# TWeber132/thesis-clip-nerf

Hardware: AMD Instinct MI355X
Metric: rendered rays/sec (64 samples/ray) at 1/2/4/8 MI355X; RGB L1 vs ref (higher is better)
Workload: dtype f32

## Files before the change

### __graft_entry__.py

```python
import os
import subprocess
import sys

ROOT = os.path.dirname(os.path.abspath(__file__))
if ROOT not in sys.path:
    sys.path.insert(0, ROOT)


def build() -> None:
    csrc = os.path.join(ROOT, 'thesis_clip_nerf_amd', 'csrc')
    subprocess.run(['make', '-C', csrc], check=True)
    subprocess.run(['make', '-C', os.path.join(ROOT, 'tests', 'cpu_math')], check=True)
    import thesis_clip_nerf_amd
    from thesis_clip_nerf_amd import _lib
    assert _lib.lib().mvnerf_abi_version() == 1


def smoke() -> None:
    import numpy as np
    import torch

    from oracle import mvnerf_oracle as O
    from thesis_clip_nerf_amd import ops
    from thesis_clip_nerf_amd.synthetic import make_scene

    dev = torch.device('cuda:0')
    sc = make_scene(seed=11, height=16, width=16, n_views=1, n_rays=64, bias_scale=0.05)
    d = {k: torch.from_numpy(np.ascontiguousarray(sc[k])).to(dev) for k in
         ['rays_o', 'rays_d', 'images', 'features', 'intrinsics', 'extrinsics_inv', 'u_coarse', 'u_fine', 'coarse', 'fine']}
    ref = O.render_call(O.unflatten_net(sc['coarse']), O.unflatten_net(sc['fine']), sc['rays_o'], sc['rays_d'],
                        sc['images'], sc['intrinsics'], sc['extrinsics_inv'], sc['features'], sc['near'], sc['far'], 64,
                        sc['u_coarse'], sc['u_fine'])
    pc, pf = ops.pack_net(d['coarse']), ops.pack_net(d['fine'])
    split = (ops.pack_net_split(d['coarse']), ops.pack_net_split(d['fine']))
    for gemm, tables in (('split_f16', 'auto'), ('split_f16', None), ('split_bf16', 'auto'), ('split_bf16', None), ('mfma_f32', 'auto'), ('mfma_f32', None)):
# ... 26 lines not shown
```

### thesis_clip_nerf_amd/csrc/field_eval_split16_impl.h

```cpp
#include <hip/hip_runtime.h>

#include "mvnerf_field_common.h"
#include "mvnerf_kernels.h"
#include "mvnerf_launch.h"
#include "mvnerf_math.h"
#include "mvnerf_mfma.h"

#ifndef MVS16_F16
#error "include through field_eval_split16.hip / field_eval_split16h.hip"
#endif
#ifndef MVS16_GUARD
#define MVS16_GUARD 0
#endif
#if MVS16_GUARD && !MVS16_F16
#error "the range guard belongs to the fp16 form: the bf16 cut has the full fp32 range"
#endif
#if MVS16_GUARD
#define MVS16_LAUNCH_FN launch_field_eval_split16h_guard
#define MVS16_KERNEL field_eval_split16h_guard_kernel
#elif MVS16_F16
#define MVS16_BYTES packed_net_split16h_bytes
#define MVS16_PACK launch_pack_net_split16h
#define MVS16_SUPPORTS field_eval_split16h_supports
#define MVS16_LAUNCH_FN launch_field_eval_split16h
#define MVS16_KERNEL field_eval_split16h_kernel
#define MVS16_PACK_KERNEL pack_net_split16h_kernel
#else
#define MVS16_BYTES packed_net_split16_bytes
#define MVS16_PACK launch_pack_net_split16
#define MVS16_SUPPORTS field_eval_split16_supports
#define MVS16_LAUNCH_FN launch_field_eval_split16
#define MVS16_KERNEL field_eval_split16_kernel
#define MVS16_PACK_KERNEL pack_net_split16_kernel
#endif

namespace mvnerf {

namespace {

using f16x2 = __attribute__((ext_vector_type(2))) _Float16;

constexpr int kS16SlotChunks = 24;
constexpr int kS16L0Pe = 2, kS16L0Feat = 8, kS16Hidden = 48;
constexpr int kS16Steps = kS16L0Pe + kS16L0Feat + kS16Hidden;
constexpr int kS16Chunks = kS16Steps * kS16SlotChunks;
constexpr int kChunkElems16 = 512;

__host__ __device__ constexpr int s16_pe_row(int g, int e) {
    return g < 3 ? 20 * g + e : (e < 12 ? 20 * (e >> 2) + 2 * (8 + ((e >> 1) & 1)) + (e & 1) : (e < 15 ? 120 + (e - 12) : -1));
}

#if !MVS16_GUARD
__global__ void MVS16_PACK_KERNEL(const float* __restrict__ src, unsigned short* __restrict__ dst) {
    const int idx = blockIdx.x * blockDim.x + threadIdx.x;
    if (idx >= kS16Chunks * kChunkElems16) return;
    const int chunk = idx / kChunkElems16, lane = (idx % kChunkElems16) / 8, jj = idx % 8;
    const int i = lane & 15, g = lane >> 4;
    const int ks = chunk / kS16SlotChunks, rb = (chunk % kS16SlotChunks) / 3, piece = chunk % 3;
    float val = 0.0f;
    if (ks < kS16L0Pe) {
        const int row = s16_pe_row(g, 8 * ks + jj);
        if (row >= 0) val = src[kKerasW0 + row * kHidden + 16 * rb + i];
    } else if (ks < kS16L0Pe + kS16L0Feat) {
        const int row = 123 + 32 * (ks - kS16L0Pe) + 8 * g + jj;
        val = src[kKerasW0 + row * kHidden + 16 * rb + i];
    } else {
        const int q = ks - kS16L0Pe - kS16L0Feat, layer = q / 4, t = q % 4;
// ... 78 lines not shown
}

__device__ __forceinline__ void pin_pieces(B16& b, int q) {
#if MVS16_F16
    unsigned u1 = b.p1[q], u3 = b.p3[q];
    asm volatile("" : "+v"(u1), "+v"(u3));
    b.p1[q] = u1;
    b.p3[q] = u3;
#else
    unsigned u1 = b.p1[q], u2 = b.p2[q], u3 = b.p3[q];
    asm volatile("" : "+v"(u1), "+v"(u2), "+v"(u3));
    b.p1[q] = u1;
    b.p2[q] = u2;
    b.p3[q] = u3;
#endif
}

template <bool kRelu>
__device__ __forceinline__ void cut8(const float (&v)[8], B16& b, RangeMax& gm, int cb) {
#pragma unroll
    for (int q = 0; q < 4; ++q) cut_pair<kRelu>(v[2 * q], v[2 * q + 1], q, b, gm, cb);
}

constexpr int kR16Slots = 3, kR16SlotF4 = kS16SlotChunks * 64;
constexpr int kS16PerView = kS16Hidden / 2;
constexpr int kS16MaxPositions = 512;

struct Ring16 {
    const f32x4* w;
    unsigned char* lds;
    int cur, nxt, fill;
    const int* table;
    int pf4, P4;
    int start_pf;
    int lane_off, wave_off;
    u32x4 a0[3];
};

__device__ __forceinline__ int ring16_start_chunk(int p, int V, int l0_units) {
    const int per_view = l0_units + kS16PerView;
    if (p < per_view * V) {
        const int q = p % per_view;
        return (q < kS16L0Pe ? q : (q < l0_units ? q : kS16L0Pe + kS16L0Feat + (q - l0_units))) * kS16SlotChunks;
    }
    return (kS16L0Pe + kS16L0Feat + kS16PerView + (p - per_view * V)) * kS16SlotChunks;
}

constexpr int kR16DmaRequests = 3;
__device__ __forceinline__ void ring16_dma(const Ring16& r, int start, int slot) {
    const unsigned char* src = reinterpret_cast<const unsigned char*>(r.w) + (unsigned)start;
    const int dst = (int)(unsigned long)(__attribute__((address_space(3))) unsigned char*)r.lds + slot + r.wave_off;
    static_assert(kR16DmaRequests * 8192 == kS16SlotChunks * 1024, "a position is kR16DmaRequests requests of 8 KiB (8 waves x 1 KiB)");
#pragma unroll
    for (int i = 0; i < kR16DmaRequests; ++i)
        asm volatile("s_mov_b32 m0, %2\n\ts_nop 0\n\tglobal_load_lds_dwordx4 %0, %1" : : "v"(r.lane_off), "s"(src + 8192 * i), "s"(dst + 8192 * i) : "memory", "m0");
}

__device__ __forceinline__ void ring16_fetch(Ring16& r) {
    ring16_dma(r, __builtin_amdgcn_readfirstlane(r.start_pf), r.fill);
    r.start_pf = *reinterpret_cast<const int*>(reinterpret_cast<const unsigned char*>(r.table) + r.pf4);
    r.pf4 = r.pf4 + 4 == r.P4 ? 0 : r.pf4 + 4;
}

__device__ __forceinline__ const f32x4* ring16_cur(const Ring16& r) { return reinterpret_cast<const f32x4*>(r.lds + r.cur); }
__device__ __forceinline__ const f32x4* ring16_nxt(const Ring16& r) { return reinterpret_cast<const f32x4*>(r.lds + r.nxt); }

__device__ __forceinline__ void ring16_next(Ring16& r) {
    __builtin_amdgcn_s_waitcnt(0x0070);
    asm volatile("s_barrier" ::: "memory");
    const int done = r.cur;
    r.cur = r.nxt;
    r.nxt = r.fill;
    r.fill = done;
}

__device__ __forceinline__ int perm_f4(int rb, int g) {
    return ((g & 1) * 64 + (rb >> 1) * 16 + 4 * (2 * (rb & 1) + (g >> 1))) >> 2;
}

template <bool kAdd>
__device__ __forceinline__ void apply_bias_row(f32x4 (&row)[2], const f32x4& bv) {
#pragma unroll
    for (int cb = 0; cb < 2; ++cb)
#pragma unroll
        for (int c = 0; c < 4; ++c) {
            if (kAdd) {
                float r = row[cb][c];
                asm("v_add_f32_e32 %0, %1, %2" : "=v"(r) : "v"(r), "v"(bv[c]));
                row[cb][c] = r;
            } else {
                row[cb][c] = bv[c];
            }
        }
}

template <bool kRelu, int kMode, bool kTailAdd, bool kInit = false>
__device__ __forceinline__ void kstep16(Ring16& ring, int lane, int g, const B16 (&b)[2], const float (&nv)[2][8], B16 (&bn)[2], f32x4 (&acc)[8][2],
                                        f32x4 (&in)[8][2], const float* __restrict__ tail_bias, RangeMax& gm, const float* __restrict__ init_bias = nullptr,
                                        f32x4 init0 = f32x4{0.0f, 0.0f, 0.0f, 0.0f}) {
    const f32x4* cur = ring16_cur(ring) + lane;
    const f32x4* nxt = ring16_nxt(ring) + lane;
    u32x4 a[3] = {ring.a0[0], ring.a0[1], ring.a0[2]};
    f32x4 bv = {0.0f, 0.0f, 0.0f, 0.0f};
    int glane = (g & 1) * 16 + (g >> 1);
    if (kMode == 4 || kInit) asm volatile("" : "+v"(glane));
    const f32x4* tail_rows = reinterpret_cast<const f32x4*>(tail_bias) + glane;
    const f32x4* init_rows = reinterpret_cast<const f32x4*>(init_bias) + glane;
    f32x4 ci = init0;
#pragma unroll
    for (int rb = 0; rb < 8; ++rb) {
        u32x4 an[3];
#pragma unroll
        for (int q = 0; q < 3; ++q) an[q] = __builtin_bit_cast(u32x4, rb < 7 ? cur[((rb + 1) * 3 + q) * 64] : nxt[q * 64]);
        if (kMode == 1) cut_pair<kRelu>(nv[rb >> 2][2 * (rb & 3)], nv[rb >> 2][2 * (rb & 3) + 1], rb & 3, bn[rb >> 2], gm, rb >> 2);
        f32x4 cin = ci;
        if (kInit && rb < 7) cin = init_rows[((rb + 1) >> 1) * 4 + 2 * ((rb + 1) & 1)];
        if (kMode == 4 && tail_bias) {
            const f32x4 bv_new = tail_rows[(rb >> 1) * 4 + 2 * (rb & 1)];
            if (rb > 0) apply_bias_row<kTailAdd>(in[rb - 1], bv);
            bv = bv_new;
        }
#if MVS16_F16
#pragma unroll
        for (int cb = 0; cb < 2; ++cb) acc[rb][cb] = mfma1632(a[1], b[cb].p3, kInit ? ci : acc[rb][cb]);
#pragma unroll
        for (int cb = 0; cb < 2; ++cb) acc[rb][cb] = mfma1632(a[2], b[cb].p1, acc[rb][cb]);
#pragma unroll
        for (int cb = 0; cb < 2; ++cb) acc[rb][cb] = mfma1632(a[0], b[cb].p1, acc[rb][cb]);
#else
#pragma unroll
        for (int cb = 0; cb < 2; ++cb) acc[rb][cb] = mfma1632(a[2], b[cb].p1, kInit ? ci : acc[rb][cb]);
#pragma unroll
        for (int cb = 0; cb < 2; ++cb) acc[rb][cb] = mfma1632(a[1], b[cb].p2, acc[rb][cb]);
#pragma unroll
        for (int cb = 0; cb < 2; ++cb) acc[rb][cb] = mfma1632(a[0], b[cb].p3, acc[rb][cb]);
#pragma unroll
        for (int cb = 0; cb < 2; ++cb) acc[rb][cb] = mfma1632(a[1], b[cb].p1, acc[rb][cb]);
#pragma unroll
        for (int cb = 0; cb < 2; ++cb) acc[rb][cb] = mfma1632(a[0], b[cb].p2, acc[rb][cb]);
#pragma unroll
        for (int cb = 0; cb < 2; ++cb) acc[rb][cb] = mfma1632(a[0], b[cb].p1, acc[rb][cb]);
#endif
        __builtin_amdgcn_sched_group_barrier(0x008, 1, 0);
        __builtin_amdgcn_sched_group_barrier(0x100, (kMode == 4 || kInit) ? 4 : 3, 0);
#pragma unroll
        for (int m = 0; m < (MVS16_F16 ? 5 : 11); ++m) {
            if (kMode == 1) __builtin_amdgcn_sched_group_barrier(0x002, MVS16_F16 ? 2 : 1, 0);
            if (kMode == 4) __builtin_amdgcn_sched_group_barrier(0x002, MVS16_F16 ? 2 : 1, 0);
            __builtin_amdgcn_sched_group_barrier(0x008, 1, 0);
        }
        if (kMode == 1) __builtin_amdgcn_sched_group_barrier(0x002, MVS16_F16 ? 3 : 2, 0);
        __builtin_amdgcn_sched_barrier(0);
        if (rb == 0) {
            asm volatile("" : "+v"(acc[0][0]), "+v"(acc[0][1]));
            ring16_fetch(ring);
            __builtin_amdgcn_sched_barrier(0);
        }
#pragma unroll
        for (int q = 0; q < 3; ++q) a[q] = an[q];
        ci = cin;
    }
#pragma unroll
    for (int q = 0; q < 3; ++q) ring.a0[q] = a[q];
    if (kMode == 4 && tail_bias) apply_bias_row<kTailAdd>(in[7], bv);
    if (kMode == 1) {
#pragma unroll
        for (int cb = 0; cb < 2; ++cb)
#pragma unroll
            for (int q = 0; q < 4; ++q) {
                pin_pieces(bn[cb], q);
            }
    }
}

__device__ __forceinline__ void first_operand_s16(const f32x4 (&in)[8][2], B16 (&b)[2], RangeMax& gm) {
#pragma unroll
    for (int cb = 0; cb < 2; ++cb) {
        const float v8[8] = {in[0][cb][0], in[0][cb][1], in[0][cb][2], in[0][cb][3], in[1][cb][0], in[1][cb][1], in[1][cb][2], in[1][cb][3]};
        cut8<true>(v8, b[cb], gm, cb);
    }
}

template <bool kTailAdd, bool kInit>
__device__ __forceinline__ void dense128_s16_plain(Ring16& ring, int lane, int g, f32x4 (&in)[8][2], f32x4 (&acc)[8][2], const float* __restrict__ tail_bias,
                                                   RangeMax& gm, const float* __restrict__ init_bias = nullptr) {
    B16 b[2], bn[2];
    f32x4 init0 = {0.0f, 0.0f, 0.0f, 0.0f};
    if (kInit) init0 = reinterpret_cast<const f32x4*>(init_bias)[perm_f4(0, g)];
    first_operand_s16(in, b, gm);
#pragma unroll
    for (int t = 0; t < 4; ++t) {
        float nv[2][8];
#pragma unroll
        for (int cb = 0; cb < 2; ++cb)
#pragma unroll
            for (int q = 0; q < 8; ++q) nv[cb][q] = t < 3 ? in[2 * (t + 1) + (q >> 2)][cb][q & 3] : 0.0f;
        if (t == 0 && kInit) kstep16<true, 1, false, true>(ring, lane, g, b, nv, bn, acc, in, nullptr, gm, init_bias, init0);
        else if (t < 3) kstep16<true, 1, false>(ring, lane, g, b, nv, bn, acc, in, nullptr, gm);
        else kstep16<true, 4, kTailAdd>(ring, lane, g, b, nv, bn, acc, in, tail_bias, gm);
        b[0] = bn[0];
        b[1] = bn[1];
        ring16_next(ring);
    }
}

template <bool kAdd>
__device__ __forceinline__ void bias16(const float* __restrict__ bperm, int g, f32x4 (&acc)[8][2]) {
    int glane = (g & 1) * 16 + (g >> 1);
    asm volatile("" : "+v"(glane));
    const f32x4* p = reinterpret_cast<const f32x4*>(bperm) + glane;
#pragma unroll
    for (int rb = 0; rb < 8; ++rb) {
        const f32x4 v = p[(rb >> 1) * 4 + 2 * (rb & 1)];
#pragma unroll
        for (int cb = 0; cb < 2; ++cb)
#pragma unroll
            for (int c = 0; c < 4; ++c) {
                if (kAdd) {
                    float r = acc[rb][cb][c];
                    asm("v_add_f32_e32 %0, %1, %2" : "=v"(r) : "v"(r), "v"(v[c]));
                    acc[rb][cb][c] = r;
                } else {
                    acc[rb][cb][c] = v[c];
                }
            }
    }
}

constexpr int kS16StageRowBytes = 256;

__device__ __forceinline__ void store_tl16(float* __restrict__ base, long tile, int n, int g, const f32x4 (&x)[8][2]) {
    const __amdgpu_buffer_rsrc_t rsrc = __builtin_amdgcn_make_buffer_rsrc(base, 0, 0xFFFFFFFF, 0x00020000);
    const int voff = (4 * g * 32 + n) * 4;
    const int tile_off = (int)((unsigned)tile * 16384u);
#pragma unroll
    for (int rb = 0; rb < 8; ++rb)
#pragma unroll
        for (int i = 0; i < 4; ++i)
#pragma unroll
            for (int cb = 0; cb < 2; ++cb) {
                const float val = x[rb][cb][i];
                __builtin_amdgcn_raw_buffer_store_b32(__builtin_bit_cast(unsigned int, val), rsrc, voff + (i * 32 + 16 * cb) * 4,
                                                      tile_off + rb * 2048, kStashAux);
            }
}

struct SampleGeo {
    long g;
    int ray, sidx, b;
    float wx, wy, wz;
    bool valid;
};

template <bool kMultiView, bool kProj, bool kAux, bool kStash>
__global__ __launch_bounds__(512, 2) void MVS16_KERNEL(FieldParams p, const f32x4* __restrict__ wsplit
#if MVS16_GUARD
                                                       , unsigned* __restrict__ range_status
#endif
) {
    constexpr int kW = 8;
    extern __shared__ __attribute__((aligned(16))) unsigned char smem_s16[];
    constexpr int kRingBytes = kR16Slots * kR16SlotF4 * 16;
    const int tid = threadIdx.x, lane = tid & 63, n = lane & 15, g = lane >> 4;
    const int wave = __builtin_amdgcn_readfirstlane(tid >> 6);
    unsigned char* stage = smem_s16 + kRingBytes + wave * (32 * kS16StageRowBytes);
    float* net = reinterpret_cast<float*>(smem_s16 + kRingBytes + kW * 32 * kS16StageRowBytes) - kPackB0;
    for (int i = tid; i < kPackBr + 8 - kPackB0; i += 64 * kW) net[kPackB0 + i] = p.net[kPackB0 + i];
    int* table = reinterpret_cast<int*>(smem_s16 + kRingBytes + kW * 32 * kS16StageRowBytes + (kPackBr + 8 - kPackB0) * 4);
    float* wr_plain = reinterpret_cast<float*>(table + kS16MaxPositions);
    for (int i = tid; i < 512; i += 64 * kW) wr_plain[i] = p.net[kPackWrPlain + i];

    Ring16 ring;
    ring.w = wsplit;
    ring.lds = smem_s16;
    ring.cur = 0;
    ring.nxt = kR16SlotF4 * 16;
    ring.fill = 2 * kR16SlotF4 * 16;
    const int l0_units = kProj ? kS16L0Pe : kS16L0Pe + kS16L0Feat;
    const int n_pos = (l0_units + kS16PerView) * p.V + kS16PerView;
    for (int i = tid; i < n_pos; i += 64 * kW) table[i] = ring16_start_chunk(i, p.V, l0_units) * 1024;
    ring.table = table;
    ring.P4 = 4 * n_pos;
    ring.pf4 = 4 * 3;
    __syncthreads();
    ring.lane_off = 16 * tid;
    ring.wave_off = 1024 * wave;
    constexpr bool kSeedHere = !kMultiView && !kAux && !kStash;
    float* seed_w = reinterpret_cast<float*>(smem_s16 + kRingBytes);
    if (kSeedHere) {
        static_assert(kPackTotal - kPackW0Dir >= 8192 && kPackB0Plain + 128 - kPackW0Dir <= 8192 && kW * 32 * kS16StageRowBytes >= 32768,
                      "four 8 KiB requests: inside the packed net, covering W0_dir and b0, inside the gather stages");
        const unsigned char* src = reinterpret_cast<const unsigned char*>(p.net + kPackW0Dir);
        const int dst = (int)(unsigned long)(__attribute__((address_space(3))) unsigned char*)seed_w + ring.wave_off;
#pragma unroll
        for (int i = 0; i < 4; ++i)
            asm volatile("s_mov_b32 m0, %2\n\ts_nop 0\n\tglobal_load_lds_dwordx4 %0, %1" : : "v"(ring.lane_off), "s"(src + 8192 * i), "s"(dst + 8192 * i) : "memory", "m0");
    }
    ring16_dma(ring, __builtin_amdgcn_readfirstlane(table[0]), ring.cur);
    ring16_dma(ring, __builtin_amdgcn_readfirstlane(table[1]), ring.nxt);
    ring.start_pf = table[2];
    if (kSeedHere) asm volatile("s_waitcnt vmcnt(%0)" : : "n"(2 * kR16DmaRequests) : "memory");
    else asm volatile("s_waitcnt vmcnt(0)" ::: "memory");
    __syncthreads();
    if (kSeedHere) {
        const unsigned last_sample = (unsigned)p.total - 1u, S = (unsigned)p.S, R = (unsigned)p.R;
        const int groups = ((int)p.n_tiles + kW - 1) / kW;
        int turn = 0;
#pragma unroll 1
        for (int grp = blockIdx.x; grp < groups; grp += gridDim.x) {
            const unsigned first = (unsigned)grp * (32u * kW), end = first + (32u * kW - 1u);
            const int ray_hi = __builtin_amdgcn_readfirstlane((int)((end < last_sample ? end : last_sample) / S));
#pragma unroll 1
            for (int ray = __builtin_amdgcn_readfirstlane((int)(first / S)); ray <= ray_hi; ++ray, ++turn)
                if ((turn & (kW - 1)) == wave) {
                    const int b = __builtin_amdgcn_readfirstlane((int)((unsigned)ray / R));
                    dir_seed_row(p, b, ray - b * (int)R, lane, seed_w);
                }
        }
        asm volatile("s_waitcnt vmcnt(0)" ::: "memory");
        __syncthreads();
    }
#pragma unroll
    for (int q = 0; q < 3; ++q) ring.a0[q] = __builtin_bit_cast(u32x4, ring16_cur(ring)[q * 64 + lane]);

    RangeMax gm;
#if MVS16_GUARD
    gm.all = 0u;
#endif
    const int n_tiles = (int)p.n_tiles, n_groups = (n_tiles + kW - 1) / kW;
    for (int grp = blockIdx.x; grp < n_groups; grp += gridDim.x) {
        const int own = grp * kW + wave;
        const bool tile_ok = own < n_tiles;
        const long tile = tile_ok ? own : n_tiles - 1;
        int pS = p.S, pR = p.R, pH = p.H, pW = p.W, gl = g, nl = n;
        asm volatile("" : "+s"(pS), "+s"(pR), "+s"(pH), "+s"(pW));
        asm volatile("" : "+v"(gl), "+v"(nl));
        SampleGeo sg[2];
        const bool one_ray = (pS & 31) == 0;
        if (one_ray) {
            const unsigned first = (unsigned)tile * 32u;
            const int ray = __builtin_amdgcn_readfirstlane((int)(first / (unsigned)pS));
            const int b = __builtin_amdgcn_readfirstlane((int)((unsigned)ray / (unsigned)pR));
            const int s0 = (int)first - ray * pS;
            const cfloat* ro = (const cfloat*)(p.rays_o + 3 * ray);
            const cfloat* rd = (const cfloat*)(p.rays_d + 3 * ray);
            const float ox = ro[0], oy = ro[1], oz = ro[2], dx = rd[0], dy = rd[1], dz = rd[2];
#pragma unroll
            for (int cb = 0; cb < 2; ++cb) {
                const long gi = (long)first + 16 * cb + nl;
                sg[cb].valid = tile_ok;
                sg[cb].g = gi;
                sg[cb].ray = ray;
                sg[cb].sidx = s0 + 16 * cb + nl;
                sg[cb].b = b;
                const float zz = p.z[gi];
                sg[cb].wx = ox + zz * dx;
// ... 6 lines not shown
                long gi = tile * 32 + 16 * cb + nl;
                sg[cb].valid = tile_ok && gi < p.total;
                if (gi >= p.total) gi = p.total - 1;
                sg[cb].g = gi;
                const int ray = (int)((unsigned)gi / (unsigned)pS);
                sg[cb].ray = ray;
                sg[cb].sidx = (int)gi - ray * pS;
                sg[cb].b = (int)((unsigned)ray / (unsigned)pR);
                const float ox = p.rays_o[3 * ray + 0], oy = p.rays_o[3 * ray + 1], oz = p.rays_o[3 * ray + 2];
                const float dx = p.rays_d[3 * ray + 0], dy = p.rays_d[3 * ray + 1], dz = p.rays_d[3 * ray + 2];
                const float zz = p.z[gi];
                sg[cb].wx = ox + zz * dx;
                sg[cb].wy = oy + zz * dy;
                sg[cb].wz = oz + zz * dz;
            }
        }

        f32x4 x[8][2], hid[8][2];
        f32x4 xsum[kMultiView ? 8 : 1][2];
#if MVS16_GUARD
        gm.cb[0] = gm.cb[1] = 0u;
#endif

        const int n_views = (kMultiView || !(kAux || kStash)) ? p.V : 1;
        for (int v = 0; v < n_views; ++v) {
            asm volatile("" : "+s"(pS), "+s"(pR), "+s"(pH), "+s"(pW));
#pragma unroll
            for (int cb = 0; cb < 2; ++cb) asm volatile("" : "+v"(sg[cb].b), "+v"(sg[cb].ray), "+v"(sg[cb].sidx));
            int tl[2];
            float ax[2], ay[2];
            long vrow[2];
            float pe[2][16];
#pragma unroll
            for (int cb = 0; cb < 2; ++cb) {
                const int bv = sg[cb].b * p.V + v;
                float cam[4], pxl, pyl;
                const f32x4* seed;
                if (one_ray) {
                    const int bu = __builtin_amdgcn_readfirstlane(sg[0].b), bvu = bu * p.V + v;
                    const int rayu = __builtin_amdgcn_readfirstlane(sg[0].ray);
                    const cfloat* Ec = (const cfloat*)(p.einv + 16 * bvu);
                    const cfloat* Kc = (const cfloat*)(p.k4 + 16 * bvu);
                    float E[16], K[12];
#pragma unroll
                    for (int i = 0; i < 16; ++i) E[i] = Ec[i];
#pragma unroll
                    for (int i = 0; i < 12; ++i) K[i] = Kc[i];
// ... 64 lines not shown
                            const float a = img[c] * 2.0f - 1.0f, bq = img[3 + c] * 2.0f - 1.0f;
                            const float cq = img[3 * pW + c] * 2.0f - 1.0f, dq = img[3 * pW + 3 + c] * 2.0f - 1.0f;
                            vb[12 + c] = bilerp(a, bq, cq, dq, tp.ax, tp.ay);
                        }
                        vb[15] = 0.0f;
                    }
#pragma unroll
                    for (int e = 0; e < 16; ++e) pe[cb][e] = gl < 3 ? va[e] : vb[e];
                }
            }

            {
                B16 bq[2], bqn[2];
#pragma unroll
                for (int cb = 0; cb < 2; ++cb) {
                    const float v8[8] = {pe[cb][0], pe[cb][1], pe[cb][2], pe[cb][3], pe[cb][4], pe[cb][5], pe[cb][6], pe[cb][7]};
                    cut8<false>(v8, bq[cb], gm, cb);
                }
                float nv[2][8];
#pragma unroll
                for (int cb = 0; cb < 2; ++cb)
#pragma unroll
                    for (int q = 0; q < 8; ++q) nv[cb][q] = pe[cb][8 + q];
                kstep16<false, 1, false>(ring, lane, g, bq, nv, bqn, x, x, nullptr, gm);
                ring16_next(ring);
                kstep16<false, 0, false>(ring, lane, g, bqn, nv, bq, x, x, nullptr, gm);
                ring16_next(ring);
            }

            asm volatile("" : "+v"(gl), "+v"(nl));
#pragma unroll
            for (int P = 0; P < (kProj ? 2 : 4); ++P) {
                asm volatile("s_waitcnt lgkmcnt(0)" ::: "memory");
                const f32x4* tbase = kProj ? reinterpret_cast<const f32x4*>(p.texel_table) + (nl >> 3) * 16 + (nl & 7) + P * 8
                                           : reinterpret_cast<const f32x4*>(p.features) + P * 16 + nl;
                const long row_f4 = kProj ? 32 : 64;
#pragma unroll
                for (int half = 0; half < 2; ++half) {
                    f32x4 tv[4][4];
                    float axs[4], ays[4];
#pragma unroll
                    for (int u = 0; u < 4; ++u) {
                        const int src = 4 * u + gl;
                        const int tls = __shfl(tl[half], src);
                        axs[u] = __shfl(ax[half], src);
                        ays[u] = __shfl(ay[half], src);
                        const f32x4* f = tbase + (long)tls * row_f4;
                        tv[u][0] = f[0];
                        tv[u][1] = f[row_f4];
                        tv[u][2] = f[(long)pW * row_f4];
                        tv[u][3] = f[(long)pW * row_f4 + row_f4];
                    }
                    __builtin_amdgcn_sched_barrier(0);
#pragma unroll
                    for (int u = 0; u < 4; ++u) {
                        const int src = 16 * half + 4 * u + gl;
                        f32x4 o;
#pragma unroll
                        for (int c = 0; c < 4; ++c) {
                            const float top = fmaf(axs[u], tv[u][1][c] - tv[u][0][c], tv[u][0][c]);
                            const float bot = fmaf(axs[u], tv[u][3][c] - tv[u][2][c], tv[u][2][c]);
                            o[c] = fmaf(ays[u], bot - top, top);
                        }
                        *reinterpret_cast<f32x4*>(stage + src * kS16StageRowBytes + ((nl ^ (src & 15)) << 4)) = o;
                    }
                }
                asm volatile("s_waitcnt lgkmcnt(0)" ::: "memory");
                if (kProj) {
#pragma unroll
                    for (int cb = 0; cb < 2; ++cb)
#pragma unroll
                        for (int rbl = 0; rbl < 4; ++rbl) {
                            const int row = 16 * cb + nl, chunk = 8 * (gl & 1) + 4 * (rbl >> 1) + 2 * (rbl & 1) + (gl >> 1);
                            const f32x4 t4 = *reinterpret_cast<const f32x4*>(stage + row * kS16StageRowBytes + ((chunk ^ (row & 15)) << 4));
#pragma unroll
                            for (int c = 0; c < 4; ++c) x[4 * P + rbl][cb][c] += t4[c];
                        }
                } else {
#pragma unroll
                    for (int s = 0; s < 2; ++s) {
                        B16 bq[2], bqn[2];
                        float nv[2][8];
#pragma unroll
                        for (int cb = 0; cb < 2; ++cb) {
                            const int row = 16 * cb + nl;
                            const f32x4 lo = *reinterpret_cast<const f32x4*>(stage + row * kS16StageRowBytes + (((8 * s + 2 * gl) ^ (row & 15)) << 4));
                            const f32x4 hi = *reinterpret_cast<const f32x4*>(stage + row * kS16StageRowBytes + (((8 * s + 2 * gl + 1) ^ (row & 15)) << 4));
                            const float b8[8] = {lo[0], lo[1], lo[2], lo[3], hi[0], hi[1], hi[2], hi[3]};
                            cut8<false>(b8, bq[cb], gm, cb);
#pragma unroll
                            for (int q = 0; q < 8; ++q) nv[cb][q] = 0.0f;
                        }
                        kstep16<false, 0, false>(ring, lane, gl, bq, nv, bqn, x, x, nullptr, gm);
                        ring16_next(ring);
                    }
                }
            }

            const long vslot = (long)p.B * p.V * p.R * p.S * 128;
            const long vtile = kMultiView ? ((long)(sg[0].b * p.V + v) * (p.n_tiles / p.B) + (tile - (long)sg[0].b * (p.n_tiles / p.B))) : tile;
            if (kStash && tile_ok) store_tl16(p.stash, vtile, n, g, x);
            auto store_acc16 = [&](float* base, const long (&rows)[2]) {
#pragma unroll
                for (int cb = 0; cb < 2; ++cb)
                    if (sg[cb].valid) {
                        float* e = base + 128 * rows[cb] + 4 * g;
#pragma unroll
                        for (int rb = 0; rb < 8; ++rb) *reinterpret_cast<f32x4*>(e + 16 * rb) = x[rb][cb];
                    }
            };
            if (kAux && p.acts_view) store_acc16(p.acts_view, vrow);
#pragma unroll 1
            for (int bi = 0; bi < 3; ++bi) {
                const float* bias1 = net + kPackBHidden + 256 * bi;
                dense128_s16_plain<true, true>(ring, lane, g, x, hid, nullptr, gm, bias1);
                if (kStash && tile_ok) store_tl16(p.stash + (1 + 2 * bi) * p.stash_stride, vtile, n, g, hid);
                bias16<true>(bias1 + 128, g, x);
                dense128_s16_plain<false, false>(ring, lane, g, hid, x, nullptr, gm);
                if (kStash && tile_ok && bi < 2) store_tl16(p.stash + (2 + 2 * bi) * p.stash_stride, vtile, n, g, x);
                if (kAux && p.acts_view) store_acc16(p.acts_view + (bi + 1) * vslot, vrow);
            }
            if (kMultiView) {
#pragma unroll
                for (int rb = 0; rb < 8; ++rb)
#pragma unroll
                    for (int cb = 0; cb < 2; ++cb) xsum[rb][cb] = (v == 0) ? x[rb][cb] : xsum[rb][cb] + x[rb][cb];
            }
        }
        if (kMultiView) {
            const float nvw = (float)p.V;
#pragma unroll
            for (int rb = 0; rb < 8; ++rb)
#pragma unroll
                for (int cb = 0; cb < 2; ++cb) x[rb][cb] = xsum[rb][cb] / nvw;
        }

        long grow[2];
        bool gvalid[2];
        {
            int ne = n;
            asm volatile("" : "+v"(ne));
#pragma unroll
            for (int cb = 0; cb < 2; ++cb) {
                long gi = tile * 32 + 16 * cb + ne;
                gvalid[cb] = tile_ok && gi < p.total;
                grow[cb] = gi >= p.total ? p.total - 1 : gi;
            }
        }
        auto store_fused16 = [&](float* base) {
#pragma unroll
            for (int cb = 0; cb < 2; ++cb)
                if (gvalid[cb]) {
                    float* e = base + 128 * grow[cb] + 4 * g;
#pragma unroll
                    for (int rb = 0; rb < 8; ++rb) *reinterpret_cast<f32x4*>(e + 16 * rb) = x[rb][cb];
                }
        };
        if (kAux && p.acts_fused) store_fused16(p.acts_fused);
        if (kStash && tile_ok) store_tl16(p.stash_fused, tile, n, g, x);
#pragma unroll 1
        for (int bi = 3; bi < 6; ++bi) {
            const float* bias1 = net + kPackBHidden + 256 * bi;
            dense128_s16_plain<true, true>(ring, lane, g, x, hid, nullptr, gm, bias1);
            if (kStash && tile_ok) store_tl16(p.stash_fused + (1 + 2 * (bi - 3)) * p.stash_fused_stride, tile, n, g, hid);
            bias16<true>(bias1 + 128, g, x);
            dense128_s16_plain<false, false>(ring, lane, g, hid, x, nullptr, gm);
            if (kStash && tile_ok) store_tl16(p.stash_fused + (2 + 2 * (bi - 3)) * p.stash_fused_stride, tile, n, g, x);
            if (kAux && p.acts_fused) store_fused16(p.acts_fused + (long)(bi - 2) * p.total * 128);
        }
        if (kAux && p.embedding) store_fused16(p.embedding);

        {
            float o[2][4] = {{0.0f, 0.0f, 0.0f, 0.0f}, {0.0f, 0.0f, 0.0f, 0.0f}};
            const f32x4* wr = reinterpret_cast<const f32x4*>(wr_plain) + 4 * g;
#pragma unroll
            for (int rb = 0; rb < 8; ++rb)
#pragma unroll
                for (int c = 0; c < 4; ++c) {
                    const f32x4 w4 = wr[16 * rb + c];
#pragma unroll
                    for (int cb = 0; cb < 2; ++cb) {
                        const float a = fmaxf(x[rb][cb][c], 0.0f);
#pragma unroll
                        for (int k = 0; k < 4; ++k) o[cb][k] = fmaf(a, w4[k], o[cb][k]);
                    }
                }
#pragma unroll
            for (int cb = 0; cb < 2; ++cb)
#pragma unroll
// ... 18 lines not shown
        }
#if MVS16_GUARD
        {
            const unsigned m0 = gvalid[0] ? gm.cb[0] : 0u, m1 = gvalid[1] ? gm.cb[1] : 0u;
            gm.all = gm.all > m0 ? gm.all : m0;
            gm.all = gm.all > m1 ? gm.all : m1;
        }
#endif
    }
    asm volatile("s_waitcnt vmcnt(0)" ::: "memory");
#if MVS16_GUARD
    {
        unsigned m = gm.all;
#pragma unroll
        for (int off = 32; off >= 1; off >>= 1) {
            const unsigned o = (unsigned)__shfl_xor((int)m, off);
            m = m > o ? m : o;
        }
        if (lane == 0) *reinterpret_cast<unsigned*>(stage) = m;
        __syncthreads();
        if (tid == 0) {
            unsigned wg = 0u;
            for (int w = 0; w < kW; ++w) {
                const unsigned o = *reinterpret_cast<const unsigned*>(smem_s16 + kRingBytes + w * (32 * kS16StageRowBytes));
                wg = wg > o ? wg : o;
            }
            atomicMax(range_status, wg);
        }
    }
#endif
}

}

#if !MVS16_GUARD
size_t MVS16_BYTES() { return (size_t)kS16Chunks * 1024; }

hipError_t MVS16_PACK(const float* net_keras, void* packed_split16, hipStream_t st) {
    const int n = kS16Chunks * kChunkElems16;
    hipLaunchKernelGGL(MVS16_PACK_KERNEL, dim3((n + 255) / 256), dim3(256), 0, st, net_keras, static_cast<unsigned short*>(packed_split16));
    return hipGetLastError();
}

bool MVS16_SUPPORTS(const FieldParams& p) {
    if (p.stash && (p.tap_idx || p.pix || p.embedding || p.acts_view || p.acts_fused)) return false;
    const int n_pos = ((p.texel_table ? kS16L0Pe : kS16L0Pe + kS16L0Feat) + kS16PerView) * p.V + kS16PerView;
    return n_pos <= kS16MaxPositions;
}
#endif

#if MVS16_GUARD
hipError_t MVS16_LAUNCH_FN(const FieldParams& p, const void* packed_split16, float* range_status, hipStream_t stream) {
    static DeviceSetup setup;
    if (!range_status || !field_eval_split16h_supports(p)) return hipErrorInvalidValue;
    unsigned* status = reinterpret_cast<unsigned*>(range_status);
#else
hipError_t MVS16_LAUNCH_FN(const FieldParams& p, const void* packed_split16, hipStream_t stream) {
    static DeviceSetup setup;
    if (!MVS16_SUPPORTS(p)) return hipErrorInvalidValue;
#endif
    const int lds_bytes = kR16Slots * kR16SlotF4 * 16 + 8 * 32 * kS16StageRowBytes + (kPackBr + 8 - kPackB0) * 4 + kS16MaxPositions * 4 + 512 * 4;
    int cus = 0;
    hipError_t e = device_setup(setup, {{&MVS16_KERNEL<false, false, false, false>, lds_bytes}, {&MVS16_KERNEL<false, true, false, false>, lds_bytes},
                                        {&MVS16_KERNEL<true, false, false, false>, lds_bytes}, {&MVS16_KERNEL<true, true, false, false>, lds_bytes},
                                        {&MVS16_KERNEL<false, false, true, false>, lds_bytes}, {&MVS16_KERNEL<false, true, true, false>, lds_bytes},
                                        {&MVS16_KERNEL<true, false, true, false>, lds_bytes}, {&MVS16_KERNEL<true, true, true, false>, lds_bytes},
                                        {&MVS16_KERNEL<false, false, false, true>, lds_bytes}, {&MVS16_KERNEL<false, true, false, true>, lds_bytes},
                                        {&MVS16_KERNEL<true, false, false, true>, lds_bytes}, {&MVS16_KERNEL<true, true, false, true>, lds_bytes}}, &cus);
    if (e != hipSuccess) return e;
    const bool mv = p.V > 1;
    const bool aux = p.tap_idx || p.pix || p.embedding || p.acts_view || p.acts_fused;
    if ((mv || aux || p.stash) && (e = launch_dir_bias(p, stream)) != hipSuccess) return e;
    const long n_groups = (p.n_tiles + 7) / 8;
    const long resident = (long)cus;
    const unsigned wgs = (unsigned)(n_groups < resident ? n_groups : resident);
    const f32x4* w = static_cast<const f32x4*>(packed_split16);
    const dim3 grid(wgs), block(512);
#if MVS16_GUARD
#define MVS16_LAUNCH(MV, PROJ, AUX, STASH) hipLaunchKernelGGL((MVS16_KERNEL<MV, PROJ, AUX, STASH>), grid, block, lds_bytes, stream, p, w, status)
#else
#define MVS16_LAUNCH(MV, PROJ, AUX, STASH) hipLaunchKernelGGL((MVS16_KERNEL<MV, PROJ, AUX, STASH>), grid, block, lds_bytes, stream, p, w)
#endif
    if (p.stash && p.V > 1 && ((long)p.R * p.S) % 32 != 0) return hipErrorInvalidValue;
    if (p.stash) {
// ... 26 lines not shown
```

Measured before the change: 4.749 million.

## Pair ring positions to halve weight-ring barriers in split16 kernel

```diff
diff --git a/__graft_entry__.py b/__graft_entry__.py
--- a/__graft_entry__.py
+++ b/__graft_entry__.py
@@ -11,6 +11,7 @@
     csrc = os.path.join(ROOT, 'thesis_clip_nerf_amd', 'csrc')
     subprocess.run(['make', '-C', csrc], check=True)
     subprocess.run(['make', '-C', os.path.join(ROOT, 'tests', 'cpu_math')], check=True)
+    subprocess.run(['make', '-C', os.path.join(ROOT, 'tests', 'cpu_ring')], check=True)
     import thesis_clip_nerf_amd
     from thesis_clip_nerf_amd import _lib
     assert _lib.lib().mvnerf_abi_version() == 1
diff --git a/thesis_clip_nerf_amd/csrc/field_eval_split16_impl.h b/thesis_clip_nerf_amd/csrc/field_eval_split16_impl.h
--- a/thesis_clip_nerf_amd/csrc/field_eval_split16_impl.h
+++ b/thesis_clip_nerf_amd/csrc/field_eval_split16_impl.h
@@ -5,6 +5,7 @@
 #include "mvnerf_launch.h"
 #include "mvnerf_math.h"
 #include "mvnerf_mfma.h"
+#include "mvnerf_ring_pairs.h"
 
 #ifndef MVS16_F16
 #error "include through field_eval_split16.hip / field_eval_split16h.hip"
@@ -43,6 +44,8 @@
 constexpr int kS16SlotChunks = 24;
 constexpr int kS16L0Pe = 2, kS16L0Feat = 8, kS16Hidden = 48;
 constexpr int kS16Steps = kS16L0Pe + kS16L0Feat + kS16Hidden;
+static_assert(kS16L0Pe % 2 == 0 && kS16L0Feat % 2 == 0 && (kS16Hidden / 2) % 2 == 0,
+              "ring positions come in pairs: layer 0's PE and feature k-steps and the k-steps of a view's blocks are all even, so every tile is");
 constexpr int kS16Chunks = kS16Steps * kS16SlotChunks;
 constexpr int kChunkElems16 = 512;
 
@@ -167,16 +170,29 @@
     for (int q = 0; q < 4; ++q) cut_pair<kRelu>(v[2 * q], v[2 * q + 1], q, b, gm, cb);
 }
 
-constexpr int kR16Slots = 3, kR16SlotF4 = kS16SlotChunks * 64;
+constexpr int kR16Slots = kRingPairSlots, kR16SlotF4 = kS16SlotChunks * 64;
+constexpr int kR16SlotBytes = kR16SlotF4 * 16;
 constexpr int kS16PerView = kS16Hidden / 2;
 constexpr int kS16MaxPositions = 512;
+
+constexpr int kS16Waves = 8;
+constexpr int kS16StageRowBytes = 256;
+constexpr int kS16StageBytes = 16 * kS16StageRowBytes;
+constexpr int kS16LdsRing = 0, kS16RingBytes = kR16Slots * kR16SlotBytes;
+constexpr int kS16LdsStage = kS16LdsRing + kS16RingBytes;
+constexpr int kS16LdsNet = kS16LdsStage + kS16Waves * kS16StageBytes;
+constexpr int kS16LdsTable = kS16LdsNet + (kPackBr + 8 - kPackB0) * 4;
+constexpr int kS16LdsWr = kS16LdsTable + kS16MaxPositions * 4;
+constexpr int kS16LdsBytes = kS16LdsWr + 512 * 4;
+static_assert(kS16LdsBytes <= 160 * 1024, "ring, gather stages, biases, position table and read-out kernel share the compute unit's 160 KiB");
+static_assert(kS16LdsStage % 16 == 0 && kS16LdsNet % 16 == 0 && kS16LdsTable % 4 == 0 && kS16LdsWr % 16 == 0, "vector accesses are aligned");
 
 struct Ring16 {
     const f32x4* w;
     unsigned char* lds;
-    int cur, nxt, fill;
+    RingSlots s;
     const int* table;
-    int pf4, P4;
+    RingCursor c;
     int start_pf;
     int lane_off, wave_off;
     u32x4 a0[3];
@@ -193,31 +209,32 @@
 
 constexpr int kR16DmaRequests = 3;
 __device__ __forceinline__ void ring16_dma(const Ring16& r, int start, int slot) {
-    const unsigned char* src = reinterpret_cast<const unsigned char*>(r.w) + (unsigned)start;
-    const int dst = (int)(unsigned long)(__attribute__((address_space(3))) unsigned char*)r.lds + slot + r.wave_off;
+    const unsigned char* src = reinterpret_cast<const unsigned char*>(r.w) + (unsigned)(start + r.wave_off);
+    const int dst = __builtin_amdgcn_readfirstlane((int)(unsigned long)(__attribute__((address_space(3))) unsigned char*)r.lds + slot + r.wave_off);
     static_assert(kR16DmaRequests * 8192 == kS16SlotChunks * 1024, "a position is kR16DmaRequests requests of 8 KiB (8 waves x 1 KiB)");
 #pragma unroll
     for (int i = 0; i < kR16DmaRequests; ++i)
         asm volatile("s_mov_b32 m0, %2\n\ts_nop 0\n\tglobal_load_lds_dwordx4 %0, %1" : : "v"(r.lane_off), "s"(src + 8192 * i), "s"(dst + 8192 * i) : "memory", "m0");
 }
 
-__device__ __forceinline__ void ring16_fetch(Ring16& r) {
-    ring16_dma(r, __builtin_amdgcn_readfirstlane(r.start_pf), r.fill);
-    r.start_pf = *reinterpret_cast<const int*>(reinterpret_cast<const unsigned char*>(r.table) + r.pf4);
-    r.pf4 = r.pf4 + 4 == r.P4 ? 0 : r.pf4 + 4;
-}
-
-__device__ __forceinline__ const f32x4* ring16_cur(const Ring16& r) { return reinterpret_cast<const f32x4*>(r.lds + r.cur); }
-__device__ __forceinline__ const f32x4* ring16_nxt(const Ring16& r) { return reinterpret_cast<const f32x4*>(r.lds + r.nxt); }
-
-__device__ __forceinline__ void ring16_next(Ring16& r) {
+__device__ __forceinline__ void ring16_fetch(Ring16& r, bool second) {
+    ring16_dma(r, __builtin_amdgcn_readfirstlane(r.start_pf), ring_slots_fill(r.s, second, kR16SlotBytes));
+    r.start_pf = *reinterpret_cast<const int*>(reinterpret_cast<const unsigned char*>(r.table) + ring_cursor_take(r.c));
+}
+
+__device__ __forceinline__ const f32x4* ring16_cur(const Ring16& r, bool second) {
+    return reinterpret_cast<const f32x4*>(r.lds + (ring_slots_cur(r.s, second, kR16SlotBytes) + r.lane_off));
+}
+__device__ __forceinline__ const f32x4* ring16_nxt(const Ring16& r, bool second) {
+    return reinterpret_cast<const f32x4*>(r.lds + (ring_slots_nxt(r.s, second, kR16SlotBytes) + r.lane_off));
+}
+
+__device__ __forceinline__ void ring16_rendezvous() {
     __builtin_amdgcn_s_waitcnt(0x0070);
     asm volatile("s_barrier" ::: "memory");
-    const int done = r.cur;
-    r.cur = r.nxt;
-    r.nxt = r.fill;
-    r.fill = done;
-}
+}
+
+__device__ __forceinline__ void ring16_next(Ring16& r, bool second) { ring_slots_advance(r.s, second); }
 
 __device__ __forceinline__ int perm_f4(int rb, int g) {
     return ((g & 1) * 64 + (rb >> 1) * 16 + 4 * (2 * (rb & 1) + (g >> 1))) >> 2;
@@ -239,12 +256,12 @@
         }
 }
 
-template <bool kRelu, int kMode, bool kTailAdd, bool kInit = false>
-__device__ __forceinline__ void kstep16(Ring16& ring, int lane, int g, const B16 (&b)[2], const float (&nv)[2][8], B16 (&bn)[2], f32x4 (&acc)[8][2],
+template <bool kPairEnd, bool kRelu, int kMode, bool kTailAdd, bool kInit = false>
+__device__ __forceinline__ void kstep16(Ring16& ring, int g, const B16 (&b)[2], const float (&nv)[2][8], B16 (&bn)[2], f32x4 (&acc)[8][2],
                                         f32x4 (&in)[8][2], const float* __restrict__ tail_bias, RangeMax& gm, const float* __restrict__ init_bias = nullptr,
                                         f32x4 init0 = f32x4{0.0f, 0.0f, 0.0f, 0.0f}) {
-    const f32x4* cur = ring16_cur(ring) + lane;
-    const f32x4* nxt = ring16_nxt(ring) + lane;
+    const f32x4* cur = ring16_cur(ring, kPairEnd);
+    const f32x4* nxt = ring16_nxt(ring, kPairEnd);
     u32x4 a[3] = {ring.a0[0], ring.a0[1], ring.a0[2]};
     f32x4 bv = {0.0f, 0.0f, 0.0f, 0.0f};
     int glane = (g & 1) * 16 + (g >> 1);
@@ -254,6 +271,10 @@
     f32x4 ci = init0;
 #pragma unroll
     for (int rb = 0; rb < 8; ++rb) {
+        if (kPairEnd && rb == 7) {
+            ring16_rendezvous();
+            __builtin_amdgcn_sched_barrier(0);
+        }
         u32x4 an[3];
 #pragma unroll
         for (int q = 0; q < 3; ++q) an[q] = __builtin_bit_cast(u32x4, rb < 7 ? cur[((rb + 1) * 3 + q) * 64] : nxt[q * 64]);
@@ -298,7 +319,7 @@
         __builtin_amdgcn_sched_barrier(0);
         if (rb == 0) {
             asm volatile("" : "+v"(acc[0][0]), "+v"(acc[0][1]));
-            ring16_fetch(ring);
+            ring16_fetch(ring, kPairEnd);
             __builtin_amdgcn_sched_barrier(0);
         }
 #pragma unroll
@@ -327,7 +348,7 @@
 }
 
 template <bool kTailAdd, bool kInit>
-__device__ __forceinline__ void dense128_s16_plain(Ring16& ring, int lane, int g, f32x4 (&in)[8][2], f32x4 (&acc)[8][2], const float* __restrict__ tail_bias,
+__device__ __forceinline__ void dense128_s16_plain(Ring16& ring, int g, f32x4 (&in)[8][2], f32x4 (&acc)[8][2], const float* __restrict__ tail_bias,
                                                    RangeMax& gm, const float* __restrict__ init_bias = nullptr) {
     B16 b[2], bn[2];
     f32x4 init0 = {0.0f, 0.0f, 0.0f, 0.0f};
@@ -340,12 +361,13 @@
         for (int cb = 0; cb < 2; ++cb)
 #pragma unroll
             for (int q = 0; q < 8; ++q) nv[cb][q] = t < 3 ? in[2 * (t + 1) + (q >> 2)][cb][q & 3] : 0.0f;
-        if (t == 0 && kInit) kstep16<true, 1, false, true>(ring, lane, g, b, nv, bn, acc, in, nullptr, gm, init_bias, init0);
-        else if (t < 3) kstep16<true, 1, false>(ring, lane, g, b, nv, bn, acc, in, nullptr, gm);
-        else kstep16<true, 4, kTailAdd>(ring, lane, g, b, nv, bn, acc, in, tail_bias, gm);
+        if (t == 0 && kInit) kstep16<false, true, 1, false, true>(ring, g, b, nv, bn, acc, in, nullptr, gm, init_bias, init0);
+        else if (t == 1) kstep16<true, true, 1, false>(ring, g, b, nv, bn, acc, in, nullptr, gm);
+        else if (t < 3) kstep16<false, true, 1, false>(ring, g, b, nv, bn, acc, in, nullptr, gm);
+        else kstep16<true, true, 4, kTailAdd>(ring, g, b, nv, bn, acc, in, tail_bias, gm);
         b[0] = bn[0];
         b[1] = bn[1];
-        ring16_next(ring);
+        ring16_next(ring, (t & 1) != 0);
     }
 }
 
@@ -372,8 +394,6 @@
     }
 }
 
-constexpr int kS16StageRowBytes = 256;
-
 __device__ __forceinline__ void store_tl16(float* __restrict__ base, long tile, int n, int g, const f32x4 (&x)[8][2]) {
     const __amdgpu_buffer_rsrc_t rsrc = __builtin_amdgcn_make_buffer_rsrc(base, 0, 0xFFFFFFFF, 0x00020000);
     const int voff = (4 * g * 32 + n) * 4;
@@ -403,46 +423,42 @@
                                                        , unsigned* __restrict__ range_status
 #endif
 ) {
-    constexpr int kW = 8;
+    constexpr int kW = kS16Waves;
     extern __shared__ __attribute__((aligned(16))) unsigned char smem_s16[];
-    constexpr int kRingBytes = kR16Slots * kR16SlotF4 * 16;
-    const int tid = threadIdx.x, lane = tid & 63, n = lane & 15, g = lane >> 4;
+    const int tid = threadIdx.x, lane = tid & 63;
     const int wave = __builtin_amdgcn_readfirstlane(tid >> 6);
-    unsigned char* stage = smem_s16 + kRingBytes + wave * (32 * kS16StageRowBytes);
-    float* net = reinterpret_cast<float*>(smem_s16 + kRingBytes + kW * 32 * kS16StageRowBytes) - kPackB0;
+    unsigned char* stage = smem_s16 + kS16LdsStage + wave * kS16StageBytes;
+    float* net = reinterpret_cast<float*>(smem_s16 + kS16LdsNet) - kPackB0;
     for (int i = tid; i < kPackBr + 8 - kPackB0; i += 64 * kW) net[kPackB0 + i] = p.net[kPackB0 + i];
-    int* table = reinterpret_cast<int*>(smem_s16 + kRingBytes + kW * 32 * kS16StageRowBytes + (kPackBr + 8 - kPackB0) * 4);
-    float* wr_plain = reinterpret_cast<float*>(table + kS16MaxPositions);
+    int* table = reinterpret_cast<int*>(smem_s16 + kS16LdsTable);
+    float* wr_plain = reinterpret_cast<float*>(smem_s16 + kS16LdsWr);
     for (int i = tid; i < 512; i += 64 * kW) wr_plain[i] = p.net[kPackWrPlain + i];
 
     Ring16 ring;
     ring.w = wsplit;
-    ring.lds = smem_s16;
-    ring.cur = 0;
-    ring.nxt = kR16SlotF4 * 16;
-    ring.fill = 2 * kR16SlotF4 * 16;
+    ring.lds = smem_s16 + kS16LdsRing;
+    ring_slots_init(ring.s, kR16SlotBytes);
     const int l0_units = kProj ? kS16L0Pe : kS16L0Pe + kS16L0Feat;
-    const int n_pos = (l0_units + kS16PerView) * p.V + kS16PerView;
+    const int n_pos = ring_pairs_positions(l0_units, kS16PerView, p.V);
     for (int i = tid; i < n_pos; i += 64 * kW) table[i] = ring16_start_chunk(i, p.V, l0_units) * 1024;
     ring.table = table;
-    ring.P4 = 4 * n_pos;
-    ring.pf4 = 4 * 3;
+    ring_cursor_init(ring.c, n_pos);
     __syncthreads();
-    ring.lane_off = 16 * tid;
+    ring.lane_off = 16 * lane;
     ring.wave_off = 1024 * wave;
     constexpr bool kSeedHere = !kMultiView && !kAux && !kStash;
-    float* seed_w = reinterpret_cast<float*>(smem_s16 + kRingBytes);
+    float* seed_w = reinterpret_cast<float*>(smem_s16 + kS16LdsStage);
     if (kSeedHere) {
-        static_assert(kPackTotal - kPackW0Dir >= 8192 && kPackB0Plain + 128 - kPackW0Dir <= 8192 && kW * 32 * kS16StageRowBytes >= 32768,
+        static_assert(kPackTotal - kPackW0Dir >= 8192 && kPackB0Plain + 128 - kPackW0Dir <= 8192 && kW * kS16StageBytes >= 32768,
                       "four 8 KiB requests: inside the packed net, covering W0_dir and b0, inside the gather stages");
-        const unsigned char* src = reinterpret_cast<const unsigned char*>(p.net + kPackW0Dir);
+        const unsigned char* src = reinterpret_cast<const unsigned char*>(p.net + kPackW0Dir) + ring.wave_off;
         const int dst = (int)(unsigned long)(__attribute__((address_space(3))) unsigned char*)seed_w + ring.wave_off;
 #pragma unroll
         for (int i = 0; i < 4; ++i)
             asm volatile("s_mov_b32 m0, %2\n\ts_nop 0\n\tglobal_load_lds_dwordx4 %0, %1" : : "v"(ring.lane_off), "s"(src + 8192 * i), "s"(dst + 8192 * i) : "memory", "m0");
     }
-    ring16_dma(ring, __builtin_amdgcn_readfirstlane(table[0]), ring.cur);
-    ring16_dma(ring, __builtin_amdgcn_readfirstlane(table[1]), ring.nxt);
+    ring16_dma(ring, __builtin_amdgcn_readfirstlane(table[0]), ring_slots_cur(ring.s, false, kR16SlotBytes));
+    ring16_dma(ring, __builtin_amdgcn_readfirstlane(table[1]), ring_slots_cur(ring.s, true, kR16SlotBytes));
     ring.start_pf = table[2];
     if (kSeedHere) asm volatile("s_waitcnt vmcnt(%0)" : : "n"(2 * kR16DmaRequests) : "memory");
     else asm volatile("s_waitcnt vmcnt(0)" ::: "memory");
@@ -466,7 +482,7 @@
         __syncthreads();
     }
 #pragma unroll
-    for (int q = 0; q < 3; ++q) ring.a0[q] = __builtin_bit_cast(u32x4, ring16_cur(ring)[q * 64 + lane]);
+    for (int q = 0; q < 3; ++q) ring.a0[q] = __builtin_bit_cast(u32x4, ring16_cur(ring, false)[q * 64]);
 
     RangeMax gm;
 #if MVS16_GUARD
@@ -477,6 +493,9 @@
         const int own = grp * kW + wave;
         const bool tile_ok = own < n_tiles;
         const long tile = tile_ok ? own : n_tiles - 1;
+        int l16 = ring.lane_off;
+        asm volatile("" : "+v"(l16));
+        const int n = (l16 >> 4) & 15, g = l16 >> 8;
         int pS = p.S, pR = p.R, pH = p.H, pW = p.W, gl = g, nl = n;
         asm volatile("" : "+s"(pS), "+s"(pR), "+s"(pH), "+s"(pW));
         asm volatile("" : "+v"(gl), "+v"(nl));
@@ -529,7 +548,7 @@
         gm.cb[0] = gm.cb[1] = 0u;
 #endif
 
-        const int n_views = (kMultiView || !(kAux || kStash)) ? p.V : 1;
+        const int n_views = kMultiView ? p.V : 1;
         for (int v = 0; v < n_views; ++v) {
             asm volatile("" : "+s"(pS), "+s"(pR), "+s"(pH), "+s"(pW));
 #pragma unroll
@@ -640,10 +659,10 @@
                 for (int cb = 0; cb < 2; ++cb)
 #pragma unroll
                     for (int q = 0; q < 8; ++q) nv[cb][q] = pe[cb][8 + q];
-                kstep16<false, 1, false>(ring, lane, g, bq, nv, bqn, x, x, nullptr, gm);
-                ring16_next(ring);
-                kstep16<false, 0, false>(ring, lane, g, bqn, nv, bq, x, x, nullptr, gm);
-                ring16_next(ring);
+                kstep16<false, false, 1, false>(ring, g, bq, nv, bqn, x, x, nullptr, gm);
+                ring16_next(ring, false);
+                kstep16<true, false, 0, false>(ring, g, bqn, nv, bq, x, x, nullptr, gm);
+                ring16_next(ring, true);
             }
 
             asm volatile("" : "+v"(gl), "+v"(nl));
@@ -653,6 +672,7 @@
                 const f32x4* tbase = kProj ? reinterpret_cast<const f32x4*>(p.texel_table) + (nl >> 3) * 16 + (nl & 7) + P * 8
                                            : reinterpret_cast<const f32x4*>(p.features) + P * 16 + nl;
                 const long row_f4 = kProj ? 32 : 64;
+                float raw[2][2][8];
 #pragma unroll
                 for (int half = 0; half < 2; ++half) {
                     f32x4 tv[4][4];
@@ -680,37 +700,45 @@
                             const float bot = fmaf(axs[u], tv[u][3][c] - tv[u][2][c], tv[u][2][c]);
                             o[c] = fmaf(ays[u], bot - top, top);
                         }
-                        *reinterpret_cast<f32x4*>(stage + src * kS16StageRowBytes + ((nl ^ (src & 15)) << 4)) = o;
+                        *reinterpret_cast<f32x4*>(stage + (src & 15) * kS16StageRowBytes + ((nl ^ (src & 15)) << 4)) = o;
                     }
-                }
-                asm volatile("s_waitcnt lgkmcnt(0)" ::: "memory");
-                if (kProj) {
-#pragma unroll
-                    for (int cb = 0; cb < 2; ++cb)
+                    asm volatile("s_waitcnt lgkmcnt(0)" ::: "memory");
+                    if (kProj) {
 #pragma unroll
                         for (int rbl = 0; rbl < 4; ++rbl) {
-                            const int row = 16 * cb + nl, chunk = 8 * (gl & 1) + 4 * (rbl >> 1) + 2 * (rbl & 1) + (gl >> 1);
-                            const f32x4 t4 = *reinterpret_cast<const f32x4*>(stage + row * kS16StageRowBytes + ((chunk ^ (row & 15)) << 4));
-#pragma unroll
-                            for (int c = 0; c < 4; ++c) x[4 * P + rbl][cb][c] += t4[c];
+                            const int chunk = 8 * (gl & 1) + 4 * (rbl >> 1) + 2 * (rbl & 1) + (gl >> 1);
+                            const f32x4 t4 = *reinterpret_cast<const f32x4*>(stage + nl * kS16StageRowBytes + ((chunk ^ nl) << 4));
+#pragma unroll
+                            for (int c = 0; c < 4; ++c) x[4 * P + rbl][half][c] += t4[c];
                         }
-                } else {
+                    } else {
+#pragma unroll
+                        for (int s = 0; s < 2; ++s) {
+                            const f32x4 lo = *reinterpret_cast<const f32x4*>(stage + nl * kS16StageRowBytes + (((8 * s + 2 * gl) ^ nl) << 4));
+                            const f32x4 hi = *reinterpret_cast<const f32x4*>(stage + nl * kS16StageRowBytes + (((8 * s + 2 * gl + 1) ^ nl) << 4));
+#pragma unroll
+                            for (int c = 0; c < 4; ++c) {
+                                raw[s][half][c] = lo[c];
+                                raw[s][half][4 + c] = hi[c];
+                            }
+                        }
+                    }
+                }
+                if (!kProj) {
+                    asm volatile("s_waitcnt lgkmcnt(0)" ::: "memory");
 #pragma unroll
                     for (int s = 0; s < 2; ++s) {
                         B16 bq[2], bqn[2];
                         float nv[2][8];
 #pragma unroll
                         for (int cb = 0; cb < 2; ++cb) {
-                            const int row = 16 * cb + nl;
-                            const f32x4 lo = *reinterpret_cast<const f32x4*>(stage + row * kS16StageRowBytes + (((8 * s + 2 * gl) ^ (row & 15)) << 4));
-                            const f32x4 hi = *reinterpret_cast<const f32x4*>(stage + row * kS16StageRowBytes + (((8 * s + 2 * gl + 1) ^ (row & 15)) << 4));
-                            const float b8[8] = {lo[0], lo[1], lo[2], lo[3], hi[0], hi[1], hi[2], hi[3]};
-                            cut8<false>(b8, bq[cb], gm, cb);
+                            cut8<false>(raw[s][cb], bq[cb], gm, cb);
 #pragma unroll
                             for (int q = 0; q < 8; ++q) nv[cb][q] = 0.0f;
                         }
-                        kstep16<false, 0, false>(ring, lane, gl, bq, nv, bqn, x, x, nullptr, gm);
-                        ring16_next(ring);
+                        if (s == 0) kstep16<false, false, 0, false>(ring, gl, bq, nv, bqn, x, x, nullptr, gm);
+                        else kstep16<true, false, 0, false>(ring, gl, bq, nv, bqn, x, x, nullptr, gm);
+                        ring16_next(ring, s != 0);
                     }
                 }
             }
@@ -731,10 +759,10 @@
 #pragma unroll 1
             for (int bi = 0; bi < 3; ++bi) {
                 const float* bias1 = net + kPackBHidden + 256 * bi;
-                dense128_s16_plain<true, true>(ring, lane, g, x, hid, nullptr, gm, bias1);
+                dense128_s16_plain<true, true>(ring, g, x, hid, nullptr, gm, bias1);
                 if (kStash && tile_ok) store_tl16(p.stash + (1 + 2 * bi) * p.stash_stride, vtile, n, g, hid);
                 bias16<true>(bias1 + 128, g, x);
-                dense128_s16_plain<false, false>(ring, lane, g, hid, x, nullptr, gm);
+                dense128_s16_plain<false, false>(ring, g, hid, x, nullptr, gm);
                 if (kStash && tile_ok && bi < 2) store_tl16(p.stash + (2 + 2 * bi) * p.stash_stride, vtile, n, g, x);
                 if (kAux && p.acts_view) store_acc16(p.acts_view + (bi + 1) * vslot, vrow);
             }
@@ -779,10 +807,10 @@
 #pragma unroll 1
         for (int bi = 3; bi < 6; ++bi) {
             const float* bias1 = net + kPackBHidden + 256 * bi;
-            dense128_s16_plain<true, true>(ring, lane, g, x, hid, nullptr, gm, bias1);
+            dense128_s16_plain<true, true>(ring, g, x, hid, nullptr, gm, bias1);
             if (kStash && tile_ok) store_tl16(p.stash_fused + (1 + 2 * (bi - 3)) * p.stash_fused_stride, tile, n, g, hid);
             bias16<true>(bias1 + 128, g, x);
-            dense128_s16_plain<false, false>(ring, lane, g, hid, x, nullptr, gm);
+            dense128_s16_plain<false, false>(ring, g, hid, x, nullptr, gm);
             if (kStash && tile_ok) store_tl16(p.stash_fused + (2 + 2 * (bi - 3)) * p.stash_fused_stride, tile, n, g, x);
             if (kAux && p.acts_fused) store_fused16(p.acts_fused + (long)(bi - 2) * p.total * 128);
         }
@@ -847,7 +875,7 @@
         if (tid == 0) {
             unsigned wg = 0u;
             for (int w = 0; w < kW; ++w) {
-                const unsigned o = *reinterpret_cast<const unsigned*>(smem_s16 + kRingBytes + w * (32 * kS16StageRowBytes));
+                const unsigned o = *reinterpret_cast<const unsigned*>(smem_s16 + kS16LdsStage + w * kS16StageBytes);
                 wg = wg > o ? wg : o;
             }
             atomicMax(range_status, wg);
@@ -869,8 +897,8 @@
 
 bool MVS16_SUPPORTS(const FieldParams& p) {
     if (p.stash && (p.tap_idx || p.pix || p.embedding || p.acts_view || p.acts_fused)) return false;
-    const int n_pos = ((p.texel_table ? kS16L0Pe : kS16L0Pe + kS16L0Feat) + kS16PerView) * p.V + kS16PerView;
-    return n_pos <= kS16MaxPositions;
+    const int n_pos = ring_pairs_positions(p.texel_table ? kS16L0Pe : kS16L0Pe + kS16L0Feat, kS16PerView, p.V);
+    return n_pos <= kS16MaxPositions && n_pos % 2 == 0;
 }
 #endif
 
@@ -884,7 +912,7 @@
     static DeviceSetup setup;
     if (!MVS16_SUPPORTS(p)) return hipErrorInvalidValue;
 #endif
-    const int lds_bytes = kR16Slots * kR16SlotF4 * 16 + 8 * 32 * kS16StageRowBytes + (kPackBr + 8 - kPackB0) * 4 + kS16MaxPositions * 4 + 512 * 4;
+    const int lds_bytes = kS16LdsBytes;
     int cus = 0;
     hipError_t e = device_setup(setup, {{&MVS16_KERNEL<false, false, false, false>, lds_bytes}, {&MVS16_KERNEL<false, true, false, false>, lds_bytes},
                                         {&MVS16_KERNEL<true, false, false, false>, lds_bytes}, {&MVS16_KERNEL<true, true, false, false>, lds_bytes},
diff --git a/thesis_clip_nerf_amd/csrc/mvnerf_ring_pairs.h b/thesis_clip_nerf_amd/csrc/mvnerf_ring_pairs.h
--- /dev/null
+++ b/thesis_clip_nerf_amd/csrc/mvnerf_ring_pairs.h
@@ -0,0 +1,59 @@
+#pragma once
+
+#if defined(__HIPCC__)
+#define MVRP_HD __host__ __device__ __forceinline__
+#else
+#define MVRP_HD static inline
+#endif
+
+namespace mvnerf {
+
+constexpr int kRingPairSlots = 4;
+
+MVRP_HD constexpr int ring_pairs_slot(int p) { return p & (kRingPairSlots - 1); }
+MVRP_HD constexpr int ring_pairs_pair(int p) { return p >> 1; }
+MVRP_HD constexpr bool ring_pairs_second(int p) { return (p & 1) != 0; }
+MVRP_HD constexpr int ring_pairs_published_by(int j) { return j + 1; }
+MVRP_HD constexpr int ring_pairs_freed_by(int j) { return j; }
+MVRP_HD constexpr int ring_pairs_fetch_position(int p) { return p + 2; }
+MVRP_HD constexpr int ring_pairs_fetch_slot(int p) { return ring_pairs_slot(p + 2); }
+
+MVRP_HD constexpr int ring_pairs_positions(int l0_units, int per_view, int views) { return (l0_units + per_view) * views + per_view; }
+
+struct RingSlots {
+    int rd, fl;
+};
+
+MVRP_HD void ring_slots_init(RingSlots& s, int stride) {
+    s.rd = 0;
+    s.fl = 2 * stride;
+}
+
+MVRP_HD int ring_slots_cur(const RingSlots& s, bool second, int stride) { return second ? s.rd + stride : s.rd; }
+MVRP_HD int ring_slots_nxt(const RingSlots& s, bool second, int stride) { return second ? s.fl : s.rd + stride; }
+MVRP_HD int ring_slots_fill(const RingSlots& s, bool second, int stride) { return second ? s.fl + stride : s.fl; }
+
+MVRP_HD void ring_slots_advance(RingSlots& s, bool second) {
+    if (second) {
+        const int done = s.rd;
+        s.rd = s.fl;
+        s.fl = done;
+    }
+}
+
+struct RingCursor {
+    int pf4, P4;
+};
+
+MVRP_HD void ring_cursor_init(RingCursor& c, int n_pos) {
+    c.P4 = 4 * n_pos;
+    c.pf4 = 4 * 3;
+}
+
+MVRP_HD int ring_cursor_take(RingCursor& c) {
+    const int at = c.pf4;
+    c.pf4 = at + 4 == c.P4 ? 0 : at + 4;
+    return at;
+}
+
+}
```

Measured after the change: 4.773 million (median of 6 runs). Within noise of the previous version (+0.5%).
